# EloDoyard/movie-recommender-system

Hardware: AMD Instinct MI355X
Metric: test-set predictions/sec (kNN k=300, fit+predict+MAE) (higher is better)
Workload: dtype fp16 MFMA similarity filter (fp32 acc) + f64 exact re-rank/prediction

## Files before the change

include/knncf.h:

```cpp
#ifndef KNNCF_H
#define KNNCF_H

#include <stdint.h>

#ifdef __cplusplus
extern "C" {
#endif

#define KNNCF_OK 0
#define KNNCF_E_INVALID (-1)
#define KNNCF_E_NONFINITE (-2)
#define KNNCF_E_DUPLICATE (-3)
#define KNNCF_E_NOMEM (-4)
#define KNNCF_E_HIP (-5)
#define KNNCF_E_STATE (-6)
#define KNNCF_E_UNSUPPORTED (-7)
#define KNNCF_E_NODEVICE (-8)

#define KNNCF_SIM_COSINE 0
#define KNNCF_SIM_ONE 1
#define KNNCF_SIM_JACCARD 2

#define KNNCF_PRED_GLOBAL_AVG 0
#define KNNCF_PRED_USER_AVG 1
#define KNNCF_PRED_ITEM_AVG 2
#define KNNCF_PRED_BASELINE 3
#define KNNCF_PRED_BASELINE_RDD 4
#define KNNCF_PRED_KNN 5
#define KNNCF_PRED_PERSONALIZED 6

#define KNNCF_FLAG_VERIFY_BOUND 1u
#define KNNCF_FLAG_BF16_FILTER 4u
#define KNNCF_FLAG_F32_PANEL 8u
#define KNNCF_FLAG_OVERLAP 2u

typedef struct knncf_handle knncf_handle;

typedef struct knncf_config {
    uint32_t struct_size;
    int32_t device;
    int32_t k;
    int32_t similarity;
    int32_t shard_rank;
    int32_t shard_count;
    int64_t workspace_bytes;
    uint32_t flags;
    uint32_t head_items;
} knncf_config;
#define KNNCF_HEAD_ALL 0xffffffffu

typedef struct knncf_timings {
    double prep_ms;
    double densify_ms;
    double gemm_ms;
    double tail_ms;
    double select_ms;
    double rerank_ms;
    double predict_ms;
    int64_t gemm_launches;
    double gemm_flops_executed;
    double gemm_flops_algorithmic;
    int64_t shortlist_total;
    int64_t fallback_rows;
    double max_bound_violation;
    int64_t head_items;
    double tail_pair_updates;
    double rerank_row_bytes;
    double select_row_bytes;
    int64_t select_launches;
} knncf_timings;

const char* knncf_version(void);
const char* knncf_status_string(int status);

int knncf_create(const knncf_config* cfg, knncf_handle** out);
void knncf_destroy(knncf_handle* h);
const char* knncf_last_error(const knncf_handle* h);

int knncf_fit(knncf_handle* h, const int32_t* users, const int32_t* items,
              const double* ratings, int64_t n);
int knncf_fit_device(knncf_handle* h, const int32_t* d_users, const int32_t* d_items,
                     const double* d_ratings, int64_t n);

int knncf_num_users(const knncf_handle* h, int32_t* out);
int knncf_num_items(const knncf_handle* h, int32_t* out);

int knncf_global_avg(knncf_handle* h, double* out);
int knncf_user_avg(knncf_handle* h, int32_t user, double* out);
int knncf_item_avg(knncf_handle* h, int32_t item, double* out);
int knncf_item_avg_dev(knncf_handle* h, int32_t item, double* out);
int knncf_item_avg_dev_rdd(knncf_handle* h, int32_t item, double* out);
int knncf_similarity(knncf_handle* h, int32_t u, int32_t v, double* out);
int knncf_knn_similarity(knncf_handle* h, int32_t u, int32_t v, double* out);
int knncf_neighbors(knncf_handle* h, int32_t u, int32_t cap, int32_t* ids, double* sims,
                    int32_t* count);
int knncf_neighbors_batch(knncf_handle* h, const int32_t* users, int64_t n, int32_t cap, int32_t* ids,
                          double* sims, int32_t* counts);
int knncf_predict(knncf_handle* h, int predictor, int32_t user, int32_t item, double* out);

int knncf_recommend(knncf_handle* h, int predictor, int32_t user, int32_t n, int32_t* items,
                    double* predictions, int32_t* count);

int knncf_recommend_batch(knncf_handle* h, int predictor, const int32_t* users, int64_t n_users, int32_t n,
                          int32_t* out_items, double* out_preds, int32_t* counts);

int knncf_query_neighbors(knncf_handle* h, int32_t user, const int32_t* items, const double* ratings, int64_t n_ratings,
                          int32_t cap, int32_t* ids, double* sims, int32_t* count);
int knncf_query_predict(knncf_handle* h, int predictor, int32_t user, const int32_t* items, const double* ratings,
                        int64_t n_ratings, const int32_t* pred_items, int64_t m, double* out);
int knncf_query_recommend(knncf_handle* h, int predictor, int32_t user, const int32_t* items, const double* ratings,
                          int64_t n_ratings, int32_t n, int32_t* out_items, double* out_preds, int32_t* count);

int knncf_query_neighbors_batch(knncf_handle* h, const int32_t* users, const int64_t* offsets, const int32_t* items,
                                const double* ratings, int64_t n_queries, int32_t cap, int32_t* ids, double* sims, int32_t* counts,
                                int32_t* statuses);
int knncf_query_predict_batch(knncf_handle* h, int predictor, const int32_t* users, const int64_t* offsets, const int32_t* items,
                              const double* ratings, int64_t n_queries, const int64_t* pred_offsets, const int32_t* pred_items,
                              double* out, int32_t* statuses);
int knncf_query_recommend_batch(knncf_handle* h, int predictor, const int32_t* users, const int64_t* offsets, const int32_t* items,
                                const double* ratings, int64_t n_queries, int32_t n, int32_t* out_items, double* out_preds,
                                int32_t* counts, int32_t* statuses);

int knncf_update_neighbors(knncf_handle* h, int32_t user, const int32_t* items, const double* ratings, int64_t n_ratings,
                           int32_t cap, int32_t* ids, double* sims, int32_t* count);
int knncf_update_predict(knncf_handle* h, int predictor, int32_t user, const int32_t* items, const double* ratings,
                         int64_t n_ratings, const int32_t* pred_items, int64_t m, double* out);
int knncf_update_recommend(knncf_handle* h, int predictor, int32_t user, const int32_t* items, const double* ratings,
                           int64_t n_ratings, int32_t n, int32_t* out_items, double* out_preds, int32_t* count);
int knncf_update_neighbors_batch(knncf_handle* h, const int32_t* users, const int64_t* offsets, const int32_t* items,
                                 const double* ratings, int64_t n_queries, int32_t cap, int32_t* ids, double* sims, int32_t* counts,
                                 int32_t* statuses);
int knncf_update_predict_batch(knncf_handle* h, int predictor, const int32_t* users, const int64_t* offsets, const int32_t* items,
                               const double* ratings, int64_t n_queries, const int64_t* pred_offsets, const int32_t* pred_items,
                               double* out, int32_t* statuses);
int knncf_update_recommend_batch(knncf_handle* h, int predictor, const int32_t* users, const int64_t* offsets, const int32_t* items,
                                 const double* ratings, int64_t n_queries, int32_t n, int32_t* out_items, double* out_preds,
                                 int32_t* counts, int32_t* statuses);

int knncf_revise_neighbors(knncf_handle* h, int32_t user, const int32_t* removed_items, int64_t n_removed, const int32_t* items,
                           const double* ratings, int64_t n_ratings, int32_t cap, int32_t* ids, double* sims, int32_t* count);
int knncf_revise_predict(knncf_handle* h, int predictor, int32_t user, const int32_t* removed_items, int64_t n_removed,
                         const int32_t* items, const double* ratings, int64_t n_ratings, const int32_t* pred_items, int64_t m,
                         double* out);
int knncf_revise_recommend(knncf_handle* h, int predictor, int32_t user, const int32_t* removed_items, int64_t n_removed,
                           const int32_t* items, const double* ratings, int64_t n_ratings, int32_t n, int32_t* out_items,
                           double* out_preds, int32_t* count);
int knncf_revise_neighbors_batch(knncf_handle* h, const int32_t* users, const int64_t* removed_offsets, const int32_t* removed_items,
                                 const int64_t* offsets, const int32_t* items, const double* ratings, int64_t n_queries, int32_t cap,
                                 int32_t* ids, double* sims, int32_t* counts, int32_t* statuses);
int knncf_revise_predict_batch(knncf_handle* h, int predictor, const int32_t* users, const int64_t* removed_offsets,
                               const int32_t* removed_items, const int64_t* offsets, const int32_t* items, const double* ratings,
                               int64_t n_queries, const int64_t* pred_offsets, const int32_t* pred_items, double* out,
                               int32_t* statuses);
int knncf_revise_recommend_batch(knncf_handle* h, int predictor, const int32_t* users, const int64_t* removed_offsets,
                                 const int32_t* removed_items, const int64_t* offsets, const int32_t* items, const double* ratings,
                                 int64_t n_queries, int32_t n, int32_t* out_items, double* out_preds, int32_t* counts,
// ... 77 lines not shown
```

movie-recommender-system_amd/csrc/predict.hip:

```cpp
#include <math.h>
#include <stdio.h>
#include <string.h>

#include "engine.h"

namespace knncf {

static constexpr int TPB = 256;
struct PredArgs {
    const int64_t* u_ptr;
    const int32_t* s_col;
    const uint32_t* s_t;
    const double* s_dev;
    const double* user_avg;
    const double* item_avg;
    const double* item_dev_hash;
    const double* item_dev_file;
    double global_avg;
    int32_t own_lo, own_hi;
    const int32_t* nbr_uidx;
    const double* nbr_usim;
    const int32_t* nbr_cnt;
    int32_t kcap;
    const int64_t* i_ptr;
// ... 263 lines not shown
        u32x2 wd[G][TR], dv[G][TR];
        uint32_t rk[G][TR], mtv[G][TR];
#pragma unroll
        for (int g = 0; g < G; ++g)
#pragma unroll
            for (int k = 0; k < TR; ++k) {
                const uint32_t wi = (rows[g] >= 0 && 64u * k + lane < (uint32_t)cur_cnt) ? bbase[g] + (x[k] >> 6) : 0x0fffffffu;
                wd[g][k] = __builtin_amdgcn_raw_buffer_load_b64(r_bits, (int)(wi * 8u), 0, 0);
                rk[g][k] = __builtin_amdgcn_raw_buffer_load_b32(r_rank, (int)(wi * 4u), 0, 0);
            }
        unsigned long long fmask[G][TR];
#pragma unroll
        for (int g = 0; g < G; ++g)
#pragma unroll
            for (int k = 0; k < TR; ++k) {
                const unsigned long long word = ((unsigned long long)wd[g][k].y << 32) | wd[g][k].x;
                const bool f = (word >> (x[k] & 63u)) & 1ull;
                fmask[g][k] = __ballot(f);
                const uint32_t q = f ? rbase[g] + rk[g][k] + (uint32_t)__popcll(word & ((1ull << (x[k] & 63u)) - 1ull)) : 0x0fffffffu;
                mtv[g][k] = __builtin_amdgcn_raw_buffer_load_b32(r_t, (int)(q * 4u), 0, 0);
                dv[g][k] = __builtin_amdgcn_raw_buffer_load_b64(r_dev, (int)(q * 8u), 0, 0);
            }
#pragma unroll
        for (int g = 0; g < G; ++g) {
            if (rows[g] < 0) continue;
            int32_t total = 0;
#pragma unroll
            for (int k = 0; k < TR; ++k) {
                const unsigned long long hit = fmask[g][k];
                if ((hit >> lane) & 1ull) {
                    const int32_t slot = total + __builtin_amdgcn_mbcnt_hi((uint32_t)(hit >> 32), __builtin_amdgcn_mbcnt_lo((uint32_t)hit, 0u));
                    mt[slot] = mtv[g][k];
                    md[slot] = __hiloint2double((int)dv[g][k].y, (int)dv[g][k].x);
                    ms[slot] = __hiloint2double((int)sv[k].y, (int)sv[k].x);
                }
                total += __popcll(hit);
            }
            for (int32_t c = total + lane; c < ((total + 3) & ~3); c += 64) mt[c] = 0xffffffffu;
            wave_sync();
            uint32_t key[TR], rank[TR];
            double kd[TR], ks[TR];
#pragma unroll
            for (int k = 0; k < TR; ++k) {
                const int32_t slot = 64 * k + lane;
                rank[k] = 0; key[k] = 0; kd[k] = 0.0; ks[k] = 0.0;
                if (slot < total) { key[k] = mt[slot]; kd[k] = md[slot]; ks[k] = ms[slot]; }
            }
            const int nslot = (total + 63) >> 6;
            const uint4* keys4 = reinterpret_cast<const uint4*>(mt);
            for (int32_t c = 0; c < ((total + 3) >> 2); ++c) {
                const uint4 kq = keys4[c];
#pragma unroll
                for (int k = 0; k < TR; ++k)
                    if (k < nslot) rank[k] += (uint32_t)(kq.x < key[k]) + (uint32_t)(kq.y < key[k]) + (uint32_t)(kq.z < key[k]) + (uint32_t)(kq.w < key[k]);
            }
#pragma unroll
            for (int k = 0; k < TR; ++k)
                if (64 * k + lane < total) { md[rank[k]] = kd[k]; ms[rank[k]] = ks[k]; }
            wave_sync();
            double num = 0.0, den = 0.0;
            for (int32_t c = 0; c < total; ++c) {
                const double sc = ms[c];
                num = num + md[c] * sc;
                den = den + fabs(sc);
            }
            wave_sync();
            const double wsd = (den > 0) ? num / den : 0.0;
            if (lane == rows[g]) my_p = combine(my_ua, wsd);
        }
    }
    if (lane < nr) {
        if (my_mine) {
            pred[my_row] = my_p;
            abs_err[my_row] = ratings ? fabs(ratings[my_row] - my_p) : 0.0;
            owned[my_row] = 1;
        } else {
            owned[my_row] = 0;
            abs_err[my_row] = 0.0;
        }
    }
}

static constexpr int PRED_CHUNK = 64;
#ifdef KNNCF_PREDICT_PROFILE
__device__ unsigned long long g_pphase[8];
#define PPH(i) do { if (threadIdx.x == 0) { const long long now_ = clock64(); atomicAdd(&g_pphase[i], (unsigned long long)(now_ - ph_t)); ph_t = now_; } } while (0)
#else
#define PPH(i) do {} while (0)
#endif
template <int TR, int G, int WAVES>
__global__ void __launch_bounds__(WAVES * 64) k_predict_knn_items(PredArgs A, int64_t n, const int32_t* __restrict__ du,
                                                              const int32_t* __restrict__ di, const double* __restrict__ ratings,
                                                              const uint32_t* __restrict__ order, double* __restrict__ pred,
                                                              double* __restrict__ abs_err, uint8_t* __restrict__ owned,
                                                              int unknown_owned) {
    constexpr int CAP = TR * 64;
    constexpr int MCAP = 64;
    constexpr int CHUNK = PRED_CHUNK;
    extern __shared__ __attribute__((aligned(16))) char smem[];
    const int ibw = (int)A.ib_words;
    const int ibw2 = (ibw + 1) >> 1;
    unsigned long long* bits = reinterpret_cast<unsigned long long*>(smem);
    uint32_t* rnk = reinterpret_cast<uint32_t*>(bits + 2 * ibw2);
    double* m_dev = reinterpret_cast<double*>(rnk + ((ibw2 + 1) & ~1));
    double* m_sim = m_dev + WAVES * MCAP;
    uint32_t* m_t = reinterpret_cast<uint32_t*>(m_sim + WAVES * MCAP);
    __shared__ int64_t s_row[CHUNK];
    __shared__ int32_t s_u[CHUNK], s_i[CHUNK], s_cnt[CHUNK];
    __shared__ uint32_t s_rb[CHUNK];
    __shared__ double s_ua[CHUNK], s_p[CHUNK];
    __shared__ uint8_t s_mine[CHUNK], s_active[CHUNK];
    const int lane = threadIdx.x & 63, wave = threadIdx.x >> 6;
    const int64_t r0 = (int64_t)blockIdx.x * CHUNK;
    if (r0 >= n) return;
    const int nr = (int)min((int64_t)CHUNK, n - r0);
#ifdef KNNCF_PREDICT_PROFILE
    long long ph_t = clock64();
#endif
    uint32_t* mt = m_t + wave * CAP;
    double* md = m_dev + wave * MCAP;
    double* ms = m_sim + wave * MCAP;
    if ((int)threadIdx.x < nr) {
        const int l = threadIdx.x;
        const int64_t row = order[r0 + l];
        const int32_t u = du[row], i = di[row];
        const bool mine = (u < 0) ? (unknown_owned != 0) : (u >= A.own_lo && u < A.own_hi);
        double ua = -1.0;
        int32_t cnt = 0;
        uint32_t rb = 0, len = 0;
        if (u >= 0) { ua = A.user_avg[u]; cnt = A.nbr_cnt[u]; }
        if (i >= 0) { rb = (uint32_t)A.i_ptr[i]; len = (uint32_t)A.i_ptr[i + 1] - rb; }
        s_row[l] = row; s_u[l] = u; s_i[l] = i; s_cnt[l] = cnt; s_rb[l] = rb; s_ua[l] = ua;
        s_p[l] = (ua < 0.0) ? A.global_avg : combine(ua, 0.0);
        s_mine[l] = mine ? 1 : 0;
        s_active[l] = (mine && ua >= 0.0 && i >= 0 && cnt > 0 && len > 0) ? 1 : 0;
    }
    __syncthreads();
    PPH(0);
    const auto r_t = __builtin_amdgcn_make_buffer_rsrc(const_cast<uint32_t*>(A.it_t), 0, A.n_bytes4, 0x00020000);
    const auto r_dev = __builtin_amdgcn_make_buffer_rsrc(const_cast<double*>(A.it_dev), 0, A.n_bytes4 * 2, 0x00020000);
    typedef __attribute__((ext_vector_type(2))) uint32_t u32x2;
    int ra = 0;
    while (ra < nr) {
        const int32_t item = s_i[ra];
        int rbn = ra + 1;
        bool any = s_active[ra] != 0;
        while (rbn < nr && s_i[rbn] == item) { any = any || s_active[rbn] != 0; ++rbn; }
        if (any) {
            const unsigned long long* gb = A.item_bits + (int64_t)item * ibw;
            const uint32_t* gr = A.item_rank + (int64_t)item * ibw;
            constexpr int NT = WAVES * 64, NB = 12;
            for (int w0 = 0; w0 < 2 * ibw2; w0 += NB * NT) {
                unsigned long long bv[NB];
                uint32_t rv[NB / 2];
#pragma unroll
                for (int q = 0; q < NB; ++q) {
                    const int w = w0 + q * NT + (int)threadIdx.x;
                    bv[q] = w < ibw ? gb[w] : 0ull;
                }
#pragma unroll
                for (int q = 0; q < NB / 2; ++q) {
                    const int j = (w0 >> 1) + q * NT + (int)threadIdx.x;
                    rv[q] = 2 * j < ibw ? gr[2 * j] : 0u;
                }
#pragma unroll
                for (int q = 0; q < NB; ++q) {
                    const int w = w0 + q * NT + (int)threadIdx.x;
                    if (w < 2 * ibw2) bits[w] = bv[q];
                }
#pragma unroll
                for (int q = 0; q < NB / 2; ++q) {
                    const int j = (w0 >> 1) + q * NT + (int)threadIdx.x;
                    if (j < ibw2) rnk[j] = rv[q];
                }
            }
            __syncthreads();
            PPH(1);
            for (int rg = ra + wave * G; rg < rbn; rg += WAVES * G) {
                int rows[G];
                int32_t cnts[G];
                uint32_t rbase[G];
                uint32_t x[G][TR];
                u32x2 sv[G][TR];
                __amdgpu_buffer_rsrc_t r_usim[G];
#pragma unroll
                for (int g = 0; g < G; ++g) {
                    const int rr = rg + g;
                    const bool on = rr < rbn && s_active[min(rr, CHUNK - 1)] != 0;
                    rows[g] = on ? rr : -1;
                    const int32_t u = __builtin_amdgcn_readfirstlane(on ? s_u[rr] : 0);
                    cnts[g] = __builtin_amdgcn_readfirstlane(on ? s_cnt[rr] : 0);
                    rbase[g] = (uint32_t)__builtin_amdgcn_readfirstlane(on ? (int)s_rb[rr] : 0);
                    const int64_t base = (int64_t)u * A.kcap;
                    const auto r_uidx = __builtin_amdgcn_make_buffer_rsrc(const_cast<int32_t*>(uniform_ptr(A.nbr_uidx + base)), 0, (uint32_t)cnts[g] * 4u, 0x00020000);
                    r_usim[g] = __builtin_amdgcn_make_buffer_rsrc(const_cast<double*>(uniform_ptr(A.nbr_usim + base)), 0, (uint32_t)cnts[g] * 8u, 0x00020000);
#pragma unroll
                    for (int k = 0; k < TR; ++k) {
                        const uint32_t j = 64u * k + lane;
                        x[g][k] = __builtin_amdgcn_raw_buffer_load_b32(r_uidx, (int)(j * 4u), 0, 0);
                    }
                }
#ifdef KNNCF_PREDICT_PROFILE
                asm volatile("s_waitcnt vmcnt(0)" ::: "memory");
                PPH(2);
#endif
                u32x2 dv[G][TR];
                uint32_t mtv[G][TR];
                unsigned long long fmask[G][TR];
#pragma unroll
                for (int g = 0; g < G; ++g)
#pragma unroll
                    for (int k = 0; k < TR; ++k) {
                        const bool have = 64 * k + lane < cnts[g];
                        const uint32_t xi = have ? x[g][k] : 0u;
                        const uint32_t wi = xi >> 6;
                        const ulonglong2 pair = *reinterpret_cast<const ulonglong2*>(bits + (wi & ~1u));
                        const unsigned long long word = (wi & 1u) ? pair.y : pair.x;
                        const bool f = have && ((word >> (xi & 63u)) & 1ull);
                        fmask[g][k] = __ballot(f);
                        const uint32_t before = rnk[wi >> 1] + ((wi & 1u) ? (uint32_t)__popcll(pair.x) : 0u);
                        const uint32_t q = f ? rbase[g] + before + (uint32_t)__popcll(word & ((1ull << (xi & 63u)) - 1ull)) : 0x0fffffffu;
                        mtv[g][k] = __builtin_amdgcn_raw_buffer_load_b32(r_t, (int)(q * 4u), 0, 0);
                        dv[g][k] = __builtin_amdgcn_raw_buffer_load_b64(r_dev, (int)(q * 8u), 0, 0);
                        sv[g][k] = __builtin_amdgcn_raw_buffer_load_b64(r_usim[g], f ? (int)((64u * k + lane) * 8u) : -1, 0, 0);
                    }
#ifdef KNNCF_PREDICT_PROFILE
                PPH(3);
                asm volatile("s_waitcnt vmcnt(0)" ::: "memory");
                PPH(4);
#endif
#pragma unroll
                for (int g = 0; g < G; ++g) {
                    if (rows[g] < 0) continue;
                    int32_t total = 0;
#pragma unroll
                    for (int k = 0; k < TR; ++k) total += __popcll(fmask[g][k]);
                    if (total == 0) continue;
                    double num = 0.0, den = 0.0;
                    if (total <= MCAP) {
                        int32_t seen = 0;
#pragma unroll
                        for (int k = 0; k < TR; ++k) {
                            const unsigned long long hit = fmask[g][k];
                            if ((hit >> lane) & 1ull) {
                                const int32_t slot = seen + __builtin_amdgcn_mbcnt_hi((uint32_t)(hit >> 32), __builtin_amdgcn_mbcnt_lo((uint32_t)hit, 0u));
                                mt[slot] = mtv[g][k];
                                md[slot] = __hiloint2double((int)dv[g][k].y, (int)dv[g][k].x);
                                ms[slot] = __hiloint2double((int)sv[g][k].y, (int)sv[g][k].x);
                            }
                            seen += __popcll(hit);
                        }
                        wave_sync();
                        uint32_t key = 0xffffffffu, rk = 0;
                        double kd = 0.0, ks = 0.0;
                        if (lane < total) { key = mt[lane]; kd = md[lane]; ks = ms[lane]; }
                        for (int32_t c = 0; c < total; ++c) rk += (uint32_t)((uint32_t)__builtin_amdgcn_readlane((int)key, c) < key);
                        if (lane < total) { md[rk] = kd; ms[rk] = ks; }
                        wave_sync();
                        for (int32_t c = 0; c < total; ++c) {
                            const double sc = ms[c];
                            num = num + md[c] * sc;
                            den = den + fabs(sc);
                        }
                        wave_sync();
                    } else {
                        int32_t seen = 0;
#pragma unroll
                        for (int k = 0; k < TR; ++k) {
                            const unsigned long long hit = fmask[g][k];
                            if ((hit >> lane) & 1ull)
                                mt[seen + __builtin_amdgcn_mbcnt_hi((uint32_t)(hit >> 32), __builtin_amdgcn_mbcnt_lo((uint32_t)hit, 0u))] = mtv[g][k];
                            seen += __popcll(hit);
                        }
                        for (int32_t c = total + lane; c < ((total + 3) & ~3); c += 64) mt[c] = 0xffffffffu;
                        wave_sync();
                        uint32_t rank[TR];
#pragma unroll
                        for (int k = 0; k < TR; ++k) rank[k] = 0;
                        const uint4* keys4 = reinterpret_cast<const uint4*>(mt);
                        for (int32_t c = 0; c < ((total + 3) >> 2); ++c) {
                            const uint4 kq = keys4[c];
#pragma unroll
                            for (int k = 0; k < TR; ++k) {
                                const uint32_t key = mtv[g][k];
                                rank[k] += (uint32_t)(kq.x < key) + (uint32_t)(kq.y < key) + (uint32_t)(kq.z < key) + (uint32_t)(kq.w < key);
                            }
                        }
                        for (int32_t b0 = 0; b0 < total; b0 += MCAP) {
#pragma unroll
                            for (int k = 0; k < TR; ++k) {
                                const uint32_t at = rank[k] - (uint32_t)b0;
                                if (((fmask[g][k] >> lane) & 1ull) && at < (uint32_t)MCAP) {
                                    md[at] = __hiloint2double((int)dv[g][k].y, (int)dv[g][k].x);
                                    ms[at] = __hiloint2double((int)sv[g][k].y, (int)sv[g][k].x);
                                }
                            }
                            wave_sync();
                            const int32_t nw = min(MCAP, total - b0);
                            for (int32_t c = 0; c < nw; ++c) {
                                const double sc = ms[c];
                                num = num + md[c] * sc;
                                den = den + fabs(sc);
                            }
                            wave_sync();
                        }
                    }
                    const double wsd = (den > 0) ? num / den : 0.0;
                    if (lane == 0) s_p[rows[g]] = combine(s_ua[rows[g]], wsd);
                }
                PPH(5);
            }
            __syncthreads();
            PPH(6);
        }
        ra = rbn;
    }
    __syncthreads();
    if ((int)threadIdx.x < nr) {
        const int l = threadIdx.x;
        const int64_t row = s_row[l];
        if (s_mine[l]) {
            const double p = s_p[l];
            pred[row] = p;
            abs_err[row] = ratings ? fabs(ratings[row] - p) : 0.0;
            owned[row] = 1;
        } else {
            owned[row] = 0;
            abs_err[row] = 0.0;
        }
    }
    PPH(7);
}

#ifdef KNNCF_PREDICT_PROFILE
static void predict_profile_dump() {
    unsigned long long h[8];
    hipMemcpyFromSymbol(h, HIP_SYMBOL(g_pphase), sizeof(h));
    unsigned long long tot = 0;
    for (int i = 0; i < 8; ++i) tot += h[i];
    static const char* names[8] = {"row data", "bitmap", "ids wait", "probe issue", "gather wait", "rank+fold", "barrier", "output"};
    fprintf(stderr, "[predict profile] total %.3e cycles:", (double)tot);
    for (int i = 0; i < 8; ++i) fprintf(stderr, " %s %.1f%%", names[i], 100.0 * (double)h[i] / (double)tot);
    fprintf(stderr, "\n");
    memset(h, 0, sizeof(h));
    hipMemcpyToSymbol(HIP_SYMBOL(g_pphase), h, sizeof(h));
}
#endif

__global__ void k_user_keys(int64_t n, const int32_t* __restrict__ du, uint32_t limit, uint64_t* __restrict__ key, uint32_t* __restrict__ val) {
    const int64_t t = (int64_t)blockIdx.x * blockDim.x + threadIdx.x;
    if (t >= n) return;
    key[t] = du[t] < 0 ? (uint64_t)limit : (uint64_t)(uint32_t)du[t];
    val[t] = (uint32_t)t;
}

__global__ void k_owned_keys(int64_t n, const int32_t* __restrict__ src, const int32_t* __restrict__ du, int32_t own_lo, int32_t own_hi,
                             int unknown_owned, uint32_t limit, uint64_t* __restrict__ key, uint32_t* __restrict__ val, unsigned long long* __restrict__ n_owned) {
    const int64_t t = (int64_t)blockIdx.x * blockDim.x + threadIdx.x;
    bool mine = false;
    if (t < n) {
        const int32_t u = du[t];
        mine = (u < 0) ? (unknown_owned != 0) : (u >= own_lo && u < own_hi);
        key[t] = !mine ? (uint64_t)limit + 1ull : (src[t] < 0 ? (uint64_t)limit : (uint64_t)(uint32_t)src[t]);
        val[t] = (uint32_t)t;
    }
    __shared__ unsigned int block_owned;
    if (threadIdx.x == 0) block_owned = 0;
    __syncthreads();
    const unsigned long long b = __ballot(mine);
    if ((threadIdx.x & 63) == 0 && b) atomicAdd(&block_owned, (unsigned int)__popcll(b));
    __syncthreads();
    if (threadIdx.x == 0 && block_owned) atomicAdd(n_owned, (unsigned long long)block_owned);
}

void launch_owned_keys(int64_t n, const int32_t* d_src, const int32_t* d_du, int32_t own_lo, int32_t own_hi, bool unknown_owned, uint32_t limit,
                       uint64_t* d_key, uint32_t* d_val, unsigned long long* d_n_owned, hipStream_t st) {
    k_owned_keys<<<(unsigned)ceil_div(n, TPB), TPB, 0, st>>>(n, d_src, d_du, own_lo, own_hi, unknown_owned ? 1 : 0, limit, d_key, d_val, d_n_owned);
    KN_HIP(hipGetLastError());
}

void launch_user_keys(int64_t n, const int32_t* d_du, uint32_t limit, uint64_t* d_key, uint32_t* d_val, hipStream_t st) {
    k_user_keys<<<(unsigned)ceil_div(n, TPB), TPB, 0, st>>>(n, d_du, limit, d_key, d_val);
    KN_HIP(hipGetLastError());
}

__global__ void k_predict_simple(PredArgs A, int kind, int64_t n, const int32_t* __restrict__ du,
                                 const int32_t* __restrict__ di, const double* __restrict__ ratings,
                                 double* __restrict__ pred, double* __restrict__ abs_err, uint8_t* __restrict__ owned,
                                 int unknown_owned) {
    int64_t t = (int64_t)blockIdx.x * blockDim.x + threadIdx.x;
    if (t >= n) return;
    const int32_t u = du[t], i = di[t];
    const bool mine = (u < 0) ? (unknown_owned != 0) : (u >= A.own_lo && u < A.own_hi);
    if (!mine) {
        owned[t] = 0;
        abs_err[t] = 0.0;
        return;
    }
    double p;
    switch (kind) {
        case KNNCF_PRED_GLOBAL_AVG: p = A.global_avg; break;
        case KNNCF_PRED_USER_AVG: p = (u >= 0) ? A.user_avg[u] : A.global_avg; break;
        case KNNCF_PRED_ITEM_AVG: p = (i >= 0) ? A.item_avg[i] : A.global_avg; break;
        default: {
            double ua = (u >= 0) ? A.user_avg[u] : -1.0;
            if (ua < 0.0) {
                p = A.global_avg;
            } else {
                double d = 0.0;
                if (i >= 0) d = (kind == KNNCF_PRED_BASELINE) ? A.item_dev_hash[i] : A.item_dev_file[i];
                p = combine(ua, d);
            }
        }
    }
    pred[t] = p;
    abs_err[t] = ratings ? fabs(ratings[t] - p) : 0.0;
    owned[t] = 1;
}

void launch_predict(const Train& tr, NeighborTable* nt, int predictor, int64_t n, const int32_t* d_du,
                    const int32_t* d_di, const double* d_ratings, const uint32_t* d_order, bool order_by_item,
                    double* d_pred, double* d_abs_err, uint8_t* d_owned, bool unknown_users_owned, hipStream_t st) {
    if (n <= 0) return;
    PredArgs A{};
    A.u_ptr = tr.u_ptr.p; A.s_col = tr.s_col.p; A.s_t = tr.s_t.p; A.s_dev = tr.s_dev.p;
    A.user_avg = tr.user_avg.p; A.item_avg = tr.item_avg.p; A.item_dev_hash = tr.item_dev_hash.p;
    A.item_dev_file = tr.item_dev_file.p; A.global_avg = tr.global_avg;
    A.own_lo = tr.own_lo; A.own_hi = tr.own_hi;
    if (predictor == KNNCF_PRED_KNN) {
        KN_REQUIRE(nt != nullptr, KNNCF_E_STATE, "predict: neighbour table missing");
        A.nbr_cnt = nt->cnt.p; A.kcap = nt->kcap;
        const bool items_path = d_order && order_by_item && tr.ib_words > 0 && lds_bitmap_fits(tr.ib_words) && nt->kcap <= 512;
        if (items_path && nt->idx.p != nullptr) {
            A.nbr_uidx = nt->idx.p; A.nbr_usim = nt->sim.p;
        } else {
            if (!nt->by_id_valid) {
                launch_sort_neighbors(*nt, tr.U, tr.U, nullptr, st);
                nt->by_id_valid = true;
            }
            A.nbr_uidx = nt->uidx.p; A.nbr_usim = nt->usim.p;
        }
        A.i_ptr = tr.i_ptr.p; A.it_user = tr.it_user.p; A.it_dev = tr.it_dev.p; A.it_t = tr.it_t.p;
        A.ib_words = tr.ib_words; A.item_bits = reinterpret_cast<const unsigned long long*>(tr.item_bits.p); A.item_rank = tr.item_rank.p;
        const double bits_total = (double)tr.I * (double)tr.ib_words * 8.0;
        if (items_path) {
            A.n_bytes4 = (uint32_t)(tr.n * 4);
            const int trips = (nt->kcap + 63) / 64;
            const unsigned blocks = (unsigned)ceil_div(n, PRED_CHUNK);
#define KN_LAUNCH_ITEMS(TRV, GV)                                                                                          \
    do {                                                                                                                  \
        const size_t ibw2 = (size_t)(tr.ib_words + 1) / 2;                                                                  \
        const size_t smem = ibw2 * 16 + ((ibw2 + 1) & ~(size_t)1) * 4 + (size_t)4 * (64 * 16 + (TRV * 64) * 4);               \
        KN_TRACE_DISPATCH("predict items TR=%d G=%d", TRV, GV);                                                           \
        KN_HIP(hipFuncSetAttribute((const void*)k_predict_knn_items<TRV, GV, 4>, hipFuncAttributeMaxDynamicSharedMemorySize, (int)smem)); \
        k_predict_knn_items<TRV, GV, 4><<<blocks, 256, smem, st>>>(A, n, d_du, d_di, d_ratings, d_order, d_pred, d_abs_err,  \
                                                                  d_owned, unknown_users_owned ? 1 : 0);                \
    } while (0)
            if (trips <= 1) KN_LAUNCH_ITEMS(1, 4);
            else if (trips <= 2) KN_LAUNCH_ITEMS(2, 4);
            else if (trips <= 4) KN_LAUNCH_ITEMS(4, 2);
            else if (trips <= 5) KN_LAUNCH_ITEMS(5, 2);
            else KN_LAUNCH_ITEMS(8, 1);
#undef KN_LAUNCH_ITEMS
            KN_HIP(hipGetLastError());
#ifdef KNNCF_PREDICT_PROFILE
            KN_HIP(hipStreamSynchronize(st));
            predict_profile_dump();
#endif
            return;
        }
        if (d_order && !order_by_item && tr.ib_words > 0 && bits_total < 4.0e9 && nt->kcap <= 512) {
            A.bits_bytes = (uint32_t)bits_total;
            A.n_bytes4 = (uint32_t)(tr.n * 4);
            const int trips = (nt->kcap + 63) / 64;
            const unsigned blocks = (unsigned)ceil_div(ceil_div(n, 32), 4);
#define KN_LAUNCH_ROWS(TRV, GV)                                                                                       \
    do {                                                                                                              \
        KN_TRACE_DISPATCH("predict rows TR=%d G=%d", TRV, GV);                                                        \
        k_predict_knn_rows<TRV, GV, 4><<<blocks, 256, 0, st>>>(A, n, d_du, d_di, d_ratings, d_order, d_pred, d_abs_err, \
                                                               d_owned, unknown_users_owned ? 1 : 0);                 \
    } while (0)
            if (trips <= 1) KN_LAUNCH_ROWS(1, 4);
            else if (trips <= 2) KN_LAUNCH_ROWS(2, 4);
            else if (trips <= 4) KN_LAUNCH_ROWS(4, 2);
            else if (trips <= 5) KN_LAUNCH_ROWS(5, 2);
            else KN_LAUNCH_ROWS(8, 1);
#undef KN_LAUNCH_ROWS
            KN_HIP(hipGetLastError());
            return;
        }
#define KN_LAUNCH_KNN(CAPV, WV)                                                                            \
    do {                                                                                                   \
        KN_TRACE_DISPATCH("predict general CAP=%d", CAPV);                                                 \
        k_predict_knn<CAPV, WV><<<(unsigned)ceil_div(n, WV), WV * 64, 0, st>>>(                              \
            A, n, d_du, d_di, d_ratings, d_order, d_pred, d_abs_err, d_owned, unknown_users_owned ? 1 : 0); \
    } while (0)
        if (nt->kcap <= 64) KN_LAUNCH_KNN(64, 4);
        else if (nt->kcap <= 128) KN_LAUNCH_KNN(128, 4);
        else if (nt->kcap <= 256) KN_LAUNCH_KNN(256, 4);
        else if (nt->kcap <= 512) KN_LAUNCH_KNN(512, 4);
        else if (nt->kcap <= 1024) KN_LAUNCH_KNN(1024, 2);
        else if (nt->kcap <= 2048) KN_LAUNCH_KNN(2048, 1);
        else throw Error(KNNCF_E_UNSUPPORTED, "predict: k > 2048 needs the tiled prediction kernel (not built yet)");
#undef KN_LAUNCH_KNN
    } else {
        k_predict_simple<<<(unsigned)ceil_div(n, TPB), TPB, 0, st>>>(A, predictor, n, d_du, d_di, d_ratings, d_pred,
                                                                     d_abs_err, d_owned, unknown_users_owned ? 1 : 0);
    }
    KN_HIP(hipGetLastError());
}

__global__ void __launch_bounds__(TPB) k_reduce_err(const double* __restrict__ abs_err, const uint8_t* __restrict__ owned,
                                                    int64_t n, double* __restrict__ partial, int64_t* __restrict__ counts) {
    __shared__ double rs[TPB];
    __shared__ long long rc[TPB];
    double s = 0.0;
    long long c = 0;
    for (int64_t t = (int64_t)blockIdx.x * TPB + threadIdx.x; t < n; t += (int64_t)gridDim.x * TPB) {
        s += abs_err[t];
        c += owned[t];
    }
    rs[threadIdx.x] = s;
    rc[threadIdx.x] = c;
    __syncthreads();
    for (int o = TPB / 2; o > 0; o >>= 1) {
        if (threadIdx.x < o) {
            rs[threadIdx.x] += rs[threadIdx.x + o];
            rc[threadIdx.x] += rc[threadIdx.x + o];
        }
        __syncthreads();
    }
    if (threadIdx.x == 0) {
        partial[blockIdx.x] = rs[0];
        counts[blockIdx.x] = rc[0];
    }
}

void launch_reduce_err(const double* d_abs_err, const uint8_t* d_owned, int64_t n, double* d_partials,
                       int64_t* d_counts, int32_t n_blocks, hipStream_t st) {
    k_reduce_err<<<n_blocks, TPB, 0, st>>>(d_abs_err, d_owned, n, d_partials, d_counts);
    KN_HIP(hipGetLastError());
}

}
```

movie-recommender-system_amd/knncf.py:

```python
import ctypes as C
import os

import numpy as np

_HERE = os.path.dirname(os.path.abspath(__file__))
LIB_PATH = os.path.join(_HERE, "libknncf.so")

OK = 0
E_INVALID, E_NONFINITE, E_DUPLICATE, E_NOMEM, E_HIP, E_STATE, E_UNSUPPORTED, E_NODEVICE, E_RCCL = range(-1, -10, -1)
SIM_COSINE, SIM_ONE, SIM_JACCARD = 0, 1, 2
PRED_GLOBAL_AVG, PRED_USER_AVG, PRED_ITEM_AVG, PRED_BASELINE, PRED_BASELINE_RDD, PRED_KNN, PRED_PERSONALIZED = range(7)
FLAG_VERIFY_BOUND = 1
FLAG_OVERLAP = 2
FLAG_BF16_FILTER = 4
FLAG_F32_PANEL = 8
HEAD_ALL = 0xFFFFFFFF

_i32p = C.POINTER(C.c_int32)
_i64p = C.POINTER(C.c_int64)
_f64p = C.POINTER(C.c_double)


class Config(C.Structure):
    _fields_ = [("struct_size", C.c_uint32), ("device", C.c_int32), ("k", C.c_int32),
                ("similarity", C.c_int32), ("shard_rank", C.c_int32), ("shard_count", C.c_int32),
                ("workspace_bytes", C.c_int64), ("flags", C.c_uint32), ("head_items", C.c_uint32)]


class Ratings(C.Structure):
    _fields_ = [("n", C.c_int64), ("users", C.POINTER(C.c_int32)), ("items", C.POINTER(C.c_int32)),
                ("ratings", C.POINTER(C.c_double))]


def load_file(path, separator="\t", threads=0, cache=None, info=None):
    L = load_library()
    r = Ratings()
    err = C.create_string_buffer(512)
    if cache is None:
        st = L.knncf_load_file(os.fsencode(path), separator.encode(), threads, C.byref(r), err, len(err))
    else:
        hit = C.c_int(0)
        st = L.knncf_load_file_cached(os.fsencode(path), separator.encode(), threads, os.fsencode(cache), C.byref(r),
                                      C.byref(hit), err, len(err))
        if info is not None:
            info["from_cache"] = bool(hit.value)
    if st != 0:
        raise KnncfError(st, err.value.decode(errors="replace"))
    try:
        n = r.n
        u = np.ctypeslib.as_array(r.users, shape=(max(n, 1),))[:n].copy()
        i = np.ctypeslib.as_array(r.items, shape=(max(n, 1),))[:n].copy()
        x = np.ctypeslib.as_array(r.ratings, shape=(max(n, 1),))[:n].copy()
    finally:
        L.knncf_free_ratings(C.byref(r))
    return u, i, x


class Personal(C.Structure):
    _fields_ = [("n_rows", C.c_int64), ("row_ids", C.POINTER(C.c_int32)), ("row_names", C.POINTER(C.c_char_p)),
                ("name_storage", C.c_void_p), ("ratings", Ratings)]


def load_personal(path, user=944):
    L = load_library()
    p = Personal()
    err = C.create_string_buffer(512)
    st = L.knncf_load_personal(os.fsencode(path), user, C.byref(p), err, len(err))
    if st != 0:
        raise KnncfError(st, err.value.decode(errors="replace"))
    try:
        names = [(int(p.row_ids[j]), p.row_names[j].decode("utf-8", errors="replace")) for j in range(p.n_rows)]
        n = p.ratings.n
        u = np.ctypeslib.as_array(p.ratings.users, shape=(max(n, 1),))[:n].copy()
        i = np.ctypeslib.as_array(p.ratings.items, shape=(max(n, 1),))[:n].copy()
        x = np.ctypeslib.as_array(p.ratings.ratings, shape=(max(n, 1),))[:n].copy()
    finally:
        L.knncf_free_personal(C.byref(p))
    return names, (u, i, x)


class Timings(C.Structure):
    _fields_ = [("prep_ms", C.c_double), ("densify_ms", C.c_double), ("gemm_ms", C.c_double),
                ("tail_ms", C.c_double), ("select_ms", C.c_double), ("rerank_ms", C.c_double), ("predict_ms", C.c_double),
                ("gemm_launches", C.c_int64), ("gemm_flops_executed", C.c_double),
                ("gemm_flops_algorithmic", C.c_double), ("shortlist_total", C.c_int64),
                ("fallback_rows", C.c_int64), ("max_bound_violation", C.c_double),
                ("head_items", C.c_int64), ("tail_pair_updates", C.c_double),
                ("rerank_row_bytes", C.c_double), ("select_row_bytes", C.c_double), ("select_launches", C.c_int64)]

    def as_dict(self):
        return {n: getattr(self, n) for n, _ in self._fields_}


class ShardView(C.Structure):
    _fields_ = [("user_begin", C.c_int32), ("user_end", C.c_int32), ("nnz_begin", C.c_int64),
                ("nnz_end", C.c_int64), ("num_users", C.c_int32), ("num_ratings", C.c_int64),
                ("d_user_avg", C.c_void_p), ("d_user_norm", C.c_void_p), ("d_dev", C.c_void_p),
                ("d_pre", C.c_void_p)]


EXPORTS = [
    "knncf_version", "knncf_status_string", "knncf_create", "knncf_destroy", "knncf_last_error",
    "knncf_fit", "knncf_fit_device", "knncf_num_users", "knncf_num_items", "knncf_global_avg",
    "knncf_user_avg", "knncf_item_avg", "knncf_item_avg_dev", "knncf_item_avg_dev_rdd", "knncf_similarity",
    "knncf_knn_similarity", "knncf_neighbors", "knncf_neighbors_batch", "knncf_predict", "knncf_recommend", "knncf_recommend_batch",
    "knncf_query_neighbors", "knncf_query_predict", "knncf_query_recommend",
    "knncf_query_neighbors_batch", "knncf_query_predict_batch", "knncf_query_recommend_batch",
    "knncf_update_neighbors", "knncf_update_predict", "knncf_update_recommend",
    "knncf_update_neighbors_batch", "knncf_update_predict_batch", "knncf_update_recommend_batch",
    "knncf_revise_neighbors", "knncf_revise_predict", "knncf_revise_recommend",
    "knncf_revise_neighbors_batch", "knncf_revise_predict_batch", "knncf_revise_recommend_batch", "knncf_predict_batch",
    "knncf_predict_batch_device", "knncf_mae", "knncf_mae_device", "knncf_mae_sweep", "knncf_mae_sweep_device", "knncf_shard_view_get",
    "knncf_shard_commit", "knncf_get_timings", "knncf_reset_timings", "knncf_reset_neighbors",
    "knncf_set_k", "knncf_load_file", "knncf_load_file_cached", "knncf_free_ratings", "knncf_load_personal", "knncf_free_personal", "knncf_neighbors_save", "knncf_neighbors_load",
    "knncf_group_create", "knncf_group_destroy", "knncf_group_last_error", "knncf_group_size", "knncf_group_handle",
    "knncf_group_fit", "knncf_group_mae", "knncf_group_predict_batch",
]


class KnncfError(RuntimeError):
    def __init__(self, status, message):
        super().__init__(f"knncf status {status}: {message}")
        self.status = status


_lib = None


def _share_hip_runtime_with_torch():
    import importlib.util

    spec = importlib.util.find_spec("torch")
    if spec is None or not spec.origin:
        return
    lib_dir = os.path.join(os.path.dirname(spec.origin), "lib")
    for name in ("libhsa-runtime64.so", "libamdhip64.so"):
        path = os.path.join(lib_dir, name)
        if os.path.exists(path):
            try:
                C.CDLL(path, mode=C.RTLD_GLOBAL)
            except OSError:
                pass


def _share_rccl_with_torch():
    import importlib.util

    if importlib.util.find_spec("torch") is not None:
        import torch


def load_library():
    global _lib
    if _lib is not None:
        return _lib
    if not os.path.exists(LIB_PATH):
        raise FileNotFoundError(
            f"{LIB_PATH} not found: build the HIP extension first (python __graft_entry__.py or "
            f"movie-recommender-system_amd/build.py); there is no CPU fallback")
    _share_hip_runtime_with_torch()
    L = C.CDLL(LIB_PATH)
    L.knncf_version.restype = C.c_char_p
    L.knncf_status_string.restype = C.c_char_p
    L.knncf_status_string.argtypes = [C.c_int]
    L.knncf_create.argtypes = [C.POINTER(Config), C.POINTER(C.c_void_p)]
    L.knncf_destroy.argtypes = [C.c_void_p]
    L.knncf_destroy.restype = None
    L.knncf_last_error.argtypes = [C.c_void_p]
    L.knncf_last_error.restype = C.c_char_p
    L.knncf_fit.argtypes = [C.c_void_p, _i32p, _i32p, _f64p, C.c_int64]
    L.knncf_fit_device.argtypes = [C.c_void_p, C.c_void_p, C.c_void_p, C.c_void_p, C.c_int64]
    L.knncf_num_users.argtypes = [C.c_void_p, _i32p]
    L.knncf_num_items.argtypes = [C.c_void_p, _i32p]
    L.knncf_global_avg.argtypes = [C.c_void_p, _f64p]
    for n in ("knncf_user_avg", "knncf_item_avg", "knncf_item_avg_dev", "knncf_item_avg_dev_rdd"):
        getattr(L, n).argtypes = [C.c_void_p, C.c_int32, _f64p]
    for n in ("knncf_similarity", "knncf_knn_similarity"):
        getattr(L, n).argtypes = [C.c_void_p, C.c_int32, C.c_int32, _f64p]
    L.knncf_neighbors.argtypes = [C.c_void_p, C.c_int32, C.c_int32, _i32p, _f64p, _i32p]
    L.knncf_neighbors_batch.argtypes = [C.c_void_p, _i32p, C.c_int64, C.c_int32, _i32p, _f64p, _i32p]
    L.knncf_predict.argtypes = [C.c_void_p, C.c_int, C.c_int32, C.c_int32, _f64p]
    L.knncf_recommend.argtypes = [C.c_void_p, C.c_int, C.c_int32, C.c_int32, _i32p, _f64p, C.POINTER(C.c_int32)]
    L.knncf_recommend_batch.argtypes = [C.c_void_p, C.c_int, _i32p, C.c_int64, C.c_int32, _i32p, _f64p, _i32p]
    for fam in ("query", "update"):
        f = lambda name: getattr(L, f"knncf_{fam}_{name}")
        f("neighbors").argtypes = [C.c_void_p, C.c_int32, _i32p, _f64p, C.c_int64, C.c_int32, _i32p, _f64p, _i32p]
        f("predict").argtypes = [C.c_void_p, C.c_int, C.c_int32, _i32p, _f64p, C.c_int64, _i32p, C.c_int64, _f64p]
        f("recommend").argtypes = [C.c_void_p, C.c_int, C.c_int32, _i32p, _f64p, C.c_int64, C.c_int32, _i32p, _f64p, _i32p]
        f("neighbors_batch").argtypes = [C.c_void_p, _i32p, _i64p, _i32p, _f64p, C.c_int64, C.c_int32, _i32p, _f64p, _i32p, _i32p]
        f("predict_batch").argtypes = [C.c_void_p, C.c_int, _i32p, _i64p, _i32p, _f64p, C.c_int64, _i64p, _i32p, _f64p, _i32p]
        f("recommend_batch").argtypes = [C.c_void_p, C.c_int, _i32p, _i64p, _i32p, _f64p, C.c_int64, C.c_int32, _i32p, _f64p,
                                         _i32p, _i32p]
    for name, at, single in (("neighbors", 2, True), ("predict", 3, True), ("recommend", 3, True),
                             ("neighbors_batch", 2, False), ("predict_batch", 3, False), ("recommend_batch", 3, False)):
        base = getattr(L, f"knncf_update_{name}").argtypes
        getattr(L, f"knncf_revise_{name}").argtypes = base[:at] + ([_i32p, C.c_int64] if single else [_i64p, _i32p]) + base[at:]
    L.knncf_predict_batch.argtypes = [C.c_void_p, C.c_int, _i32p, _i32p, C.c_int64, _f64p]
    L.knncf_predict_batch_device.argtypes = [C.c_void_p, C.c_int, C.c_void_p, C.c_void_p, C.c_int64, C.c_void_p]
    L.knncf_mae.argtypes = [C.c_void_p, C.c_int, _i32p, _i32p, _f64p, C.c_int64, _f64p]
    L.knncf_mae_device.argtypes = [C.c_void_p, C.c_int, C.c_void_p, C.c_void_p, C.c_void_p, C.c_int64,
                                   _f64p, C.POINTER(C.c_int64), C.c_void_p]
    L.knncf_mae_sweep.argtypes = [C.c_void_p, _i32p, C.c_int32, _i32p, _i32p, _f64p, C.c_int64, _f64p, _f64p]
    L.knncf_mae_sweep_device.argtypes = [C.c_void_p, _i32p, C.c_int32, C.c_void_p, C.c_void_p, C.c_void_p, C.c_int64, _f64p,
                                         C.POINTER(C.c_int64), C.c_void_p]
    L.knncf_shard_view_get.argtypes = [C.c_void_p, C.POINTER(ShardView)]
    L.knncf_shard_commit.argtypes = [C.c_void_p]
    L.knncf_get_timings.argtypes = [C.c_void_p, C.POINTER(Timings)]
    L.knncf_reset_timings.argtypes = [C.c_void_p]
    L.knncf_reset_neighbors.argtypes = [C.c_void_p]
    L.knncf_set_k.argtypes = [C.c_void_p, C.c_int32]
    L.knncf_load_file.argtypes = [C.c_char_p, C.c_char_p, C.c_int, C.POINTER(Ratings), C.c_char_p, C.c_int]
    L.knncf_load_file_cached.argtypes = [C.c_char_p, C.c_char_p, C.c_int, C.c_char_p, C.POINTER(Ratings), C.POINTER(C.c_int),
                                         C.c_char_p, C.c_int]
    L.knncf_free_ratings.argtypes = [C.POINTER(Ratings)]
    L.knncf_free_ratings.restype = None
    L.knncf_load_personal.argtypes = [C.c_char_p, C.c_int32, C.POINTER(Personal), C.c_char_p, C.c_int]
    L.knncf_free_personal.argtypes = [C.POINTER(Personal)]
    L.knncf_free_personal.restype = None
    L.knncf_neighbors_save.argtypes = [C.c_void_p, C.c_char_p]
    L.knncf_neighbors_load.argtypes = [C.c_void_p, C.c_char_p]
    L.knncf_group_create.argtypes = [C.POINTER(Config), _i32p, C.c_int32, C.POINTER(C.c_void_p)]
    L.knncf_group_destroy.argtypes = [C.c_void_p]
    L.knncf_group_destroy.restype = None
    L.knncf_group_last_error.argtypes = [C.c_void_p]
    L.knncf_group_last_error.restype = C.c_char_p
    L.knncf_group_size.argtypes = [C.c_void_p, _i32p]
    L.knncf_group_handle.argtypes = [C.c_void_p, C.c_int32, C.POINTER(C.c_void_p)]
    L.knncf_group_fit.argtypes = [C.c_void_p, _i32p, _i32p, _f64p, C.c_int64]
    L.knncf_group_mae.argtypes = [C.c_void_p, C.c_int, _i32p, _i32p, _f64p, C.c_int64, _f64p]
    L.knncf_group_predict_batch.argtypes = [C.c_void_p, C.c_int, _i32p, _i32p, C.c_int64, _f64p]
    _lib = L
    return L


def _i32(a):
    return np.ascontiguousarray(a, dtype=np.int32)


def _f64(a):
    return np.ascontiguousarray(a, dtype=np.float64)


def _dev_ptr(t, dtype_name):
    import torch

    want = {"int32": torch.int32, "float64": torch.float64}[dtype_name]
    if not t.is_cuda or t.dtype != want or not t.is_contiguous():
# ... 505 lines not shown
```

Baseline: 85.64 million.

## Shrink predict-items LDS footprint and raise occupancy with windowed match staging

Reduces the per-wave shared-memory staging in the item prediction kernel from a TR*64 key array plus 64-entry buffers to a 32-entry window. Matches are now processed in up to two windows, and the large-match path ranks keys with cross-lane readlane instead of an LDS key array. Per-row shared state is compacted (flags byte, 32-bit row, 16-bit count, user average folded into s_p), launch bounds request 5 blocks per CU, and lane offsets are precomputed. The aim is more resident blocks per CU by cutting LDS and register pressure. The cost is extra wave syncs and window loops for rows with 33-64 matches, and a readlane loop whose length grows with the match count.

```diff
diff --git a/include/knncf.h b/include/knncf.h
--- a/include/knncf.h
+++ b/include/knncf.h
@@ -72,6 +72,7 @@
 
 const char* knncf_version(void);
 const char* knncf_status_string(int status);
+int64_t knncf_predict_items_lds_bytes(int64_t n_users);
 
 int knncf_create(const knncf_config* cfg, knncf_handle** out);
 void knncf_destroy(knncf_handle* h);
diff --git a/movie-recommender-system_amd/csrc/predict.hip b/movie-recommender-system_amd/csrc/predict.hip
--- a/movie-recommender-system_amd/csrc/predict.hip
+++ b/movie-recommender-system_amd/csrc/predict.hip
@@ -369,6 +369,11 @@
 }
 
 static constexpr int PRED_CHUNK = 64;
+static constexpr int PRED_MCAP = 32;
+static inline size_t pred_items_lds_bytes(int64_t ib_words, int waves) {
+    const size_t ibw2 = (size_t)(ib_words + 1) / 2;
+    return ibw2 * 16 + ((ibw2 + 1) & ~(size_t)1) * 4 + (size_t)waves * PRED_MCAP * (8 + 8 + 4);
+}
 #ifdef KNNCF_PREDICT_PROFILE
 __device__ unsigned long long g_pphase[8];
 #define PPH(i) do { if (threadIdx.x == 0) { const long long now_ = clock64(); atomicAdd(&g_pphase[i], (unsigned long long)(now_ - ph_t)); ph_t = now_; } } while (0)
@@ -376,40 +381,38 @@
 #define PPH(i) do {} while (0)
 #endif
 template <int TR, int G, int WAVES>
-__global__ void __launch_bounds__(WAVES * 64) k_predict_knn_items(PredArgs A, int64_t n, const int32_t* __restrict__ du,
+__global__ void __launch_bounds__(WAVES * 64, 5) k_predict_knn_items(PredArgs A, int64_t n, const int32_t* __restrict__ du,
                                                               const int32_t* __restrict__ di, const double* __restrict__ ratings,
                                                               const uint32_t* __restrict__ order, double* __restrict__ pred,
                                                               double* __restrict__ abs_err, uint8_t* __restrict__ owned,
                                                               int unknown_owned) {
-    constexpr int CAP = TR * 64;
-    constexpr int MCAP = 64;
+    constexpr int MCAP = PRED_MCAP;
     constexpr int CHUNK = PRED_CHUNK;
+    static_assert(MCAP <= 32 && CHUNK <= 256, "a lane holds one match of up to two windows; one thread per row");
     extern __shared__ __attribute__((aligned(16))) char smem[];
     const int ibw = (int)A.ib_words;
     const int ibw2 = (ibw + 1) >> 1;
     unsigned long long* bits = reinterpret_cast<unsigned long long*>(smem);
     uint32_t* rnk = reinterpret_cast<uint32_t*>(bits + 2 * ibw2);
-    double* m_dev = reinterpret_cast<double*>(rnk + ((ibw2 + 1) & ~1));
-    double* m_sim = m_dev + WAVES * MCAP;
-    uint32_t* m_t = reinterpret_cast<uint32_t*>(m_sim + WAVES * MCAP);
-    __shared__ int64_t s_row[CHUNK];
-    __shared__ int32_t s_u[CHUNK], s_i[CHUNK], s_cnt[CHUNK];
-    __shared__ uint32_t s_rb[CHUNK];
-    __shared__ double s_ua[CHUNK], s_p[CHUNK];
-    __shared__ uint8_t s_mine[CHUNK], s_active[CHUNK];
-    const int lane = threadIdx.x & 63, wave = threadIdx.x >> 6;
+    double* m_win = reinterpret_cast<double*>(rnk + ((ibw2 + 1) & ~1));
+    __shared__ double s_p[CHUNK];
+    __shared__ int32_t s_u[CHUNK], s_i[CHUNK];
+    __shared__ uint32_t s_row[CHUNK], s_rb[CHUNK];
+    __shared__ uint16_t s_cnt[CHUNK];
+    __shared__ uint8_t s_flags[CHUNK];
+    const int lane = threadIdx.x & 63, wave = __builtin_amdgcn_readfirstlane((int)(threadIdx.x >> 6));
     const int64_t r0 = (int64_t)blockIdx.x * CHUNK;
     if (r0 >= n) return;
     const int nr = (int)min((int64_t)CHUNK, n - r0);
 #ifdef KNNCF_PREDICT_PROFILE
     long long ph_t = clock64();
 #endif
-    uint32_t* mt = m_t + wave * CAP;
-    double* md = m_dev + wave * MCAP;
-    double* ms = m_sim + wave * MCAP;
+    double* md = m_win + wave * (MCAP * 5 / 2);
+    double* ms = md + MCAP;
+    uint32_t* mt = reinterpret_cast<uint32_t*>(ms + MCAP);
     if ((int)threadIdx.x < nr) {
         const int l = threadIdx.x;
-        const int64_t row = order[r0 + l];
+        const uint32_t row = order[r0 + l];
         const int32_t u = du[row], i = di[row];
         const bool mine = (u < 0) ? (unknown_owned != 0) : (u >= A.own_lo && u < A.own_hi);
         double ua = -1.0;
@@ -417,10 +420,10 @@
         uint32_t rb = 0, len = 0;
         if (u >= 0) { ua = A.user_avg[u]; cnt = A.nbr_cnt[u]; }
         if (i >= 0) { rb = (uint32_t)A.i_ptr[i]; len = (uint32_t)A.i_ptr[i + 1] - rb; }
-        s_row[l] = row; s_u[l] = u; s_i[l] = i; s_cnt[l] = cnt; s_rb[l] = rb; s_ua[l] = ua;
-        s_p[l] = (ua < 0.0) ? A.global_avg : combine(ua, 0.0);
-        s_mine[l] = mine ? 1 : 0;
-        s_active[l] = (mine && ua >= 0.0 && i >= 0 && cnt > 0 && len > 0) ? 1 : 0;
+        const bool active = mine && ua >= 0.0 && i >= 0 && cnt > 0 && len > 0;
+        s_row[l] = row; s_u[l] = u; s_i[l] = i; s_cnt[l] = (uint16_t)cnt; s_rb[l] = rb;
+        s_p[l] = active ? ua : (ua < 0.0) ? A.global_avg : combine(ua, 0.0);
+        s_flags[l] = (mine ? 1 : 0) | (active ? 2 : 0);
     }
     __syncthreads();
     PPH(0);
@@ -431,8 +434,8 @@
     while (ra < nr) {
         const int32_t item = s_i[ra];
         int rbn = ra + 1;
-        bool any = s_active[ra] != 0;
-        while (rbn < nr && s_i[rbn] == item) { any = any || s_active[rbn] != 0; ++rbn; }
+        bool any = (s_flags[ra] & 2) != 0;
+        while (rbn < nr && s_i[rbn] == item) { any = any || (s_flags[rbn] & 2) != 0; ++rbn; }
         if (any) {
             const unsigned long long* gb = A.item_bits + (int64_t)item * ibw;
             const uint32_t* gr = A.item_rank + (int64_t)item * ibw;
@@ -464,6 +467,9 @@
             __syncthreads();
             PPH(1);
             for (int rg = ra + wave * G; rg < rbn; rg += WAVES * G) {
+                uint32_t lane4, lane8;
+                asm volatile("v_lshlrev_b32 %0, 2, %1" : "=v"(lane4) : "v"(lane));
+                asm volatile("v_lshlrev_b32 %0, 3, %1" : "=v"(lane8) : "v"(lane));
                 int rows[G];
                 int32_t cnts[G];
                 uint32_t rbase[G];
@@ -473,18 +479,17 @@
 #pragma unroll
                 for (int g = 0; g < G; ++g) {
                     const int rr = rg + g;
-                    const bool on = rr < rbn && s_active[min(rr, CHUNK - 1)] != 0;
+                    const bool on = rr < rbn && (s_flags[min(rr, CHUNK - 1)] & 2) != 0;
                     rows[g] = on ? rr : -1;
                     const int32_t u = __builtin_amdgcn_readfirstlane(on ? s_u[rr] : 0);
-                    cnts[g] = __builtin_amdgcn_readfirstlane(on ? s_cnt[rr] : 0);
+                    cnts[g] = __builtin_amdgcn_readfirstlane(on ? (int)s_cnt[rr] : 0);
                     rbase[g] = (uint32_t)__builtin_amdgcn_readfirstlane(on ? (int)s_rb[rr] : 0);
                     const int64_t base = (int64_t)u * A.kcap;
                     const auto r_uidx = __builtin_amdgcn_make_buffer_rsrc(const_cast<int32_t*>(uniform_ptr(A.nbr_uidx + base)), 0, (uint32_t)cnts[g] * 4u, 0x00020000);
                     r_usim[g] = __builtin_amdgcn_make_buffer_rsrc(const_cast<double*>(uniform_ptr(A.nbr_usim + base)), 0, (uint32_t)cnts[g] * 8u, 0x00020000);
 #pragma unroll
                     for (int k = 0; k < TR; ++k) {
-                        const uint32_t j = 64u * k + lane;
-                        x[g][k] = __builtin_amdgcn_raw_buffer_load_b32(r_uidx, (int)(j * 4u), 0, 0);
+                        x[g][k] = __builtin_amdgcn_raw_buffer_load_b32(r_uidx, (int)(lane4 + 256u * k), 0, 0);
                     }
                 }
 #ifdef KNNCF_PREDICT_PROFILE
@@ -498,7 +503,7 @@
                 for (int g = 0; g < G; ++g)
 #pragma unroll
                     for (int k = 0; k < TR; ++k) {
-                        const bool have = 64 * k + lane < cnts[g];
+                        const bool have = (int32_t)lane4 < 4 * (cnts[g] - 64 * k);
                         const uint32_t xi = have ? x[g][k] : 0u;
                         const uint32_t wi = xi >> 6;
                         const ulonglong2 pair = *reinterpret_cast<const ulonglong2*>(bits + (wi & ~1u));
@@ -509,7 +514,7 @@
                         const uint32_t q = f ? rbase[g] + before + (uint32_t)__popcll(word & ((1ull << (xi & 63u)) - 1ull)) : 0x0fffffffu;
                         mtv[g][k] = __builtin_amdgcn_raw_buffer_load_b32(r_t, (int)(q * 4u), 0, 0);
                         dv[g][k] = __builtin_amdgcn_raw_buffer_load_b64(r_dev, (int)(q * 8u), 0, 0);
-                        sv[g][k] = __builtin_amdgcn_raw_buffer_load_b64(r_usim[g], f ? (int)((64u * k + lane) * 8u) : -1, 0, 0);
+                        sv[g][k] = __builtin_amdgcn_raw_buffer_load_b64(r_usim[g], (int)((f ? lane8 : 0x7ffff000u) + 512u * k), 0, 0);
                     }
 #ifdef KNNCF_PREDICT_PROFILE
                 PPH(3);
@@ -522,55 +527,51 @@
                     int32_t total = 0;
 #pragma unroll
                     for (int k = 0; k < TR; ++k) total += __popcll(fmask[g][k]);
-                    if (total == 0) continue;
                     double num = 0.0, den = 0.0;
-                    if (total <= MCAP) {
-                        int32_t seen = 0;
-#pragma unroll
-                        for (int k = 0; k < TR; ++k) {
-                            const unsigned long long hit = fmask[g][k];
-                            if ((hit >> lane) & 1ull) {
-                                const int32_t slot = seen + __builtin_amdgcn_mbcnt_hi((uint32_t)(hit >> 32), __builtin_amdgcn_mbcnt_lo((uint32_t)hit, 0u));
-                                mt[slot] = mtv[g][k];
-                                md[slot] = __hiloint2double((int)dv[g][k].y, (int)dv[g][k].x);
-                                ms[slot] = __hiloint2double((int)sv[g][k].y, (int)sv[g][k].x);
-                            }
-                            seen += __popcll(hit);
-                        }
-                        wave_sync();
+                    if (total > 0 && total <= 2 * MCAP) {
                         uint32_t key = 0xffffffffu, rk = 0;
                         double kd = 0.0, ks = 0.0;
-                        if (lane < total) { key = mt[lane]; kd = md[lane]; ks = ms[lane]; }
+                        for (int32_t b0 = 0; b0 < total; b0 += MCAP) {
+                            int32_t seen = -b0;
+#pragma unroll
+                            for (int k = 0; k < TR; ++k) {
+                                const unsigned long long hit = fmask[g][k];
+                                const uint32_t slot = (uint32_t)(seen + (int32_t)__builtin_amdgcn_mbcnt_hi((uint32_t)(hit >> 32), __builtin_amdgcn_mbcnt_lo((uint32_t)hit, 0u)));
+                                if (((hit >> lane) & 1ull) && slot < (uint32_t)MCAP) {
+                                    mt[slot] = mtv[g][k];
+                                    md[slot] = __hiloint2double((int)dv[g][k].y, (int)dv[g][k].x);
+                                    ms[slot] = __hiloint2double((int)sv[g][k].y, (int)sv[g][k].x);
+                                }
+                                seen += __popcll(hit);
+                            }
+                            wave_sync();
+                            const uint32_t at = (uint32_t)(lane - b0);
+                            if (at < (uint32_t)MCAP && lane < total) { key = mt[at]; kd = md[at]; ks = ms[at]; }
+                            wave_sync();
+                        }
                         for (int32_t c = 0; c < total; ++c) rk += (uint32_t)((uint32_t)__builtin_amdgcn_readlane((int)key, c) < key);
-                        if (lane < total) { md[rk] = kd; ms[rk] = ks; }
-                        wave_sync();
-                        for (int32_t c = 0; c < total; ++c) {
-                            const double sc = ms[c];
-                            num = num + md[c] * sc;
-                            den = den + fabs(sc);
+                        for (int32_t b0 = 0; b0 < total; b0 += MCAP) {
+                            const uint32_t at = rk - (uint32_t)b0;
+                            if (lane < total && at < (uint32_t)MCAP) { md[at] = kd; ms[at] = ks; }
+                            wave_sync();
+                            const int32_t nw = min(MCAP, total - b0);
+                            for (int32_t c = 0; c < nw; ++c) {
+                                const double sc = ms[c];
+                                num = num + md[c] * sc;
+                                den = den + fabs(sc);
+                            }
+                            wave_sync();
                         }
-                        wave_sync();
-                    } else {
-                        int32_t seen = 0;
-#pragma unroll
-                        for (int k = 0; k < TR; ++k) {
-                            const unsigned long long hit = fmask[g][k];
-                            if ((hit >> lane) & 1ull)
-                                mt[seen + __builtin_amdgcn_mbcnt_hi((uint32_t)(hit >> 32), __builtin_amdgcn_mbcnt_lo((uint32_t)hit, 0u))] = mtv[g][k];
-                            seen += __popcll(hit);
-                        }
-                        for (int32_t c = total + lane; c < ((total + 3) & ~3); c += 64) mt[c] = 0xffffffffu;
-                        wave_sync();
+                    } else if (total > 0) {
                         uint32_t rank[TR];
 #pragma unroll
                         for (int k = 0; k < TR; ++k) rank[k] = 0;
-                        const uint4* keys4 = reinterpret_cast<const uint4*>(mt);
-                        for (int32_t c = 0; c < ((total + 3) >> 2); ++c) {
-                            const uint4 kq = keys4[c];
-#pragma unroll
-                            for (int k = 0; k < TR; ++k) {
-                                const uint32_t key = mtv[g][k];
-                                rank[k] += (uint32_t)(kq.x < key) + (uint32_t)(kq.y < key) + (uint32_t)(kq.z < key) + (uint32_t)(kq.w < key);
+#pragma unroll
+                        for (int k2 = 0; k2 < TR; ++k2) {
+                            for (unsigned long long m = fmask[g][k2]; m != 0ull; m &= m - 1ull) {
+                                const uint32_t other = (uint32_t)__builtin_amdgcn_readlane((int)mtv[g][k2], __builtin_ctzll(m));
+#pragma unroll
+                                for (int k = 0; k < TR; ++k) rank[k] += (uint32_t)(other < mtv[g][k]);
                             }
                         }
                         for (int32_t b0 = 0; b0 < total; b0 += MCAP) {
@@ -593,7 +594,7 @@
                         }
                     }
                     const double wsd = (den > 0) ? num / den : 0.0;
-                    if (lane == 0) s_p[rows[g]] = combine(s_ua[rows[g]], wsd);
+                    if (lane == 0) s_p[rows[g]] = combine(s_p[rows[g]], wsd);
                 }
                 PPH(5);
             }
@@ -606,7 +607,7 @@
     if ((int)threadIdx.x < nr) {
         const int l = threadIdx.x;
         const int64_t row = s_row[l];
-        if (s_mine[l]) {
+        if (s_flags[l] & 1) {
             const double p = s_p[l];
             pred[row] = p;
             abs_err[row] = ratings ? fabs(ratings[row] - p) : 0.0;
@@ -736,8 +737,7 @@
             const unsigned blocks = (unsigned)ceil_div(n, PRED_CHUNK);
 #define KN_LAUNCH_ITEMS(TRV, GV)                                                                                          \
     do {                                                                                                                  \
-        const size_t ibw2 = (size_t)(tr.ib_words + 1) / 2;                                                                  \
-        const size_t smem = ibw2 * 16 + ((ibw2 + 1) & ~(size_t)1) * 4 + (size_t)4 * (64 * 16 + (TRV * 64) * 4);               \
+        const size_t smem = pred_items_lds_bytes(tr.ib_words, 4);                                                        \
         KN_TRACE_DISPATCH("predict items TR=%d G=%d", TRV, GV);                                                           \
         KN_HIP(hipFuncSetAttribute((const void*)k_predict_knn_items<TRV, GV, 4>, hipFuncAttributeMaxDynamicSharedMemorySize, (int)smem)); \
         k_predict_knn_items<TRV, GV, 4><<<blocks, 256, smem, st>>>(A, n, d_du, d_di, d_ratings, d_order, d_pred, d_abs_err,  \
@@ -830,3 +830,7 @@
 }
 
 }
+
+extern "C" int64_t knncf_predict_items_lds_bytes(int64_t n_users) {
+    return (int64_t)knncf::pred_items_lds_bytes((n_users + 63) / 64, 4);
+}
diff --git a/movie-recommender-system_amd/knncf.py b/movie-recommender-system_amd/knncf.py
--- a/movie-recommender-system_amd/knncf.py
+++ b/movie-recommender-system_amd/knncf.py
@@ -100,7 +100,7 @@
 
 
 EXPORTS = [
-    "knncf_version", "knncf_status_string", "knncf_create", "knncf_destroy", "knncf_last_error",
+    "knncf_version", "knncf_status_string", "knncf_predict_items_lds_bytes", "knncf_create", "knncf_destroy", "knncf_last_error",
     "knncf_fit", "knncf_fit_device", "knncf_num_users", "knncf_num_items", "knncf_global_avg",
     "knncf_user_avg", "knncf_item_avg", "knncf_item_avg_dev", "knncf_item_avg_dev_rdd", "knncf_similarity",
     "knncf_knn_similarity", "knncf_neighbors", "knncf_neighbors_batch", "knncf_predict", "knncf_recommend", "knncf_recommend_batch",
@@ -163,6 +163,8 @@
     L.knncf_version.restype = C.c_char_p
     L.knncf_status_string.restype = C.c_char_p
     L.knncf_status_string.argtypes = [C.c_int]
+    L.knncf_predict_items_lds_bytes.restype = C.c_int64
+    L.knncf_predict_items_lds_bytes.argtypes = [C.c_int64]
     L.knncf_create.argtypes = [C.POINTER(Config), C.POINTER(C.c_void_p)]
     L.knncf_destroy.argtypes = [C.c_void_p]
     L.knncf_destroy.restype = None
```

After: 86.18 million (median of 6 runs). About the same (+0.6%).
